# raulmur/ORB_SLAM2

Measured on NVIDIA H100. Metric: stereo frames/sec (ORB extract L+R + ComputeStereoMatches, KITTI-shaped 1242x375 @2000 kpts), higher is better.
Workload: dtype u8

## Files before the change

### orb_slam2_b200/csrc/borb_host.cu

```cuda
#include <cmath>
#include <cstdarg>
#include <cstdio>
#include <algorithm>
#include <cstdlib>
#include <cstring>

#include "borb_internal.h"

namespace borb {

static thread_local std::string tl_error;
void set_error(const char* fmt, ...) {
    char buf[512];
    va_list ap;
    va_start(ap, fmt);
    vsnprintf(buf, sizeof(buf), fmt, ap);
    va_end(ap);
    tl_error = buf;
}

bool allow_max_smem(const void* func) {
    static std::mutex mu;
    static std::vector<std::pair<const void*, int>> done;
    int dev = 0;
// ... 66 lines not shown
        int r = 2 * dst - 2 - (dst + k);
        if (r < 0) r = 0;
        for (int j = 0; j < 4; j++) out.push_back(out[first + (size_t)r * 4 + j]);
    }
    if (((out.size() - first) / 4) & 1) for (int j = 0; j < 4; j++) out.push_back(0);
}

bool resize_window_table(const std::vector<int16_t>& tabs, size_t xtab_first, int n_entries, std::vector<int16_t>& out) {
    bool ok = true;
    for (int gq = 0; gq < n_entries; gq += 4) {
        int lo = 1 << 30, hi = 0;
        for (int i = 0; i < 4; i++) {
            const int ofs = tabs[xtab_first + (size_t)(gq + i) * 4];
            lo = std::min(lo, ofs); hi = std::max(hi, ofs);
        }
        const int base = lo & ~3;
        if (hi + 1 - base > 11) ok = false;
        for (int i = 0; i < 4; i++) {
            const int16_t* e = &tabs[xtab_first + (size_t)(gq + i) * 4];
            const int pos = e[0] - base;
            int s1 = 0, s2 = 0x10;
            if (pos <= 6) s1 = pos | ((pos + 1) << 4);
            else if (pos == 7) { s1 = 7; s2 = 0x40; }
            else { const int q = (pos - 8) + 4; s2 = q | ((q + 1) << 4); }
            out.push_back(e[1]);
            out.push_back(e[2]);
            out.push_back((int16_t)base);
            out.push_back((int16_t)((s1 | (s2 << 8)) & 0x7FFF));
        }
    }
    return ok;
}

const int8_t kPattern[1024] = {
#include "orb_pattern.inc"
};

borb_status build_geometry(borb_extractor* e, int w, int h, std::vector<int16_t>& tabs) {
    Geometry& g = e->geom;
    std::memset(&g, 0, sizeof(g));
    const int L = e->cfg.n_levels;
    g.nlevels = L; g.w = w; g.h = h;
    g.fast_mode = e->fast_mode;
    g.ini_th = e->cfg.ini_th_fast < 0 ? 0 : (e->cfg.ini_th_fast > 255 ? 255 : e->cfg.ini_th_fast);
    g.min_th = e->cfg.min_th_fast < 0 ? 0 : (e->cfg.min_th_fast > 255 ? 255 : e->cfg.min_th_fast);
    for (int i = 0; i < 16; i++) g.umax[i] = e->umax[i];
    unsigned pyr_off = 0, cand_off = 0;
    int blk = 0, sel_off = 0, btile = 0;
    tabs.clear();
    for (int l = 0; l < L; l++) {
        LevelGeom& v = g.lv[l];
        v.w = cv_round_f((float)w * e->inv_scale[l]);
        v.h = cv_round_f((float)h * e->inv_scale[l]);
        const float width = (float)(v.w - 2 * MIN_BORDER), height = (float)(v.h - 2 * MIN_BORDER);
        v.nCols = (int)(width / 30.f);
        v.nRows = (int)(height / 30.f);
        if (v.nCols < 1 || v.nRows < 1) {
            set_error("level %d is %dx%d: too small for the 30-px FAST cell grid (reference divides by zero)", l, v.w, v.h);
            return BORB_ERR_UNSUPPORTED;
        }
        v.wCell = (int)std::ceil(width / v.nCols);
        v.hCell = (int)std::ceil(height / v.nRows);
        v.pitch = align_up(v.w + 8, 128);
        v.pyr_off = pyr_off;
        pyr_off += (unsigned)v.pitch * v.h;
        v.cellsPerBlk = FAST_TILE_W / v.wCell > 0 ? FAST_TILE_W / v.wCell : 1;
        v.rowsPerBlk = fast_rows_per_blk(v.nRows, v.hCell);
        v.blkCols = (v.nCols + v.cellsPerBlk - 1) / v.cellsPerBlk;
        v.blkBase = blk;
        blk += v.blkCols * ((v.nRows + v.rowsPerBlk - 1) / v.rowsPerBlk);
        v.cand_off = cand_off;
        v.cand_cap = v.nCols * v.nRows * ((v.wCell + 1) / 2) * ((v.hCell + 1) / 2);
        cand_off += (unsigned)align_up(v.cand_cap, 32);
        v.quota = e->per_level[l];
        v.nIni = (int)std::round(width / height);
        if (v.nIni < 1) { set_error("level %d aspect ratio gives zero quadtree roots (reference divides by zero)", l); return BORB_ERR_UNSUPPORTED; }
        v.hX = width / v.nIni;
        v.node_cap = (v.quota > 4 * v.nIni ? v.quota : 4 * v.nIni) + 3;
        v.node_cap = align_up(v.node_cap + 1, 4);
        v.sel_off = sel_off;
        sel_off += v.node_cap;
        v.scale = e->scale[l];
        v.inv_scale = e->inv_scale[l];
        v.patch_size = (float)(int)(PATCH * e->scale[l]);
        g.blur_base[l] = btile;
        btile += ((v.w + BLUR_TILE_W - 1) / BLUR_TILE_W) * ((v.h + BLUR_TILE_H - 1) / BLUR_TILE_H);
        if (l > 0) {
            const int wpad = (v.w + 8 + 3) & ~3;
            v.xtab_off = (unsigned)(tabs.size() / 4);
            resize_table(g.lv[l - 1].w, v.w, true, wpad - v.w, tabs);
            v.ytab_off = (unsigned)(tabs.size() / 4);
            resize_table(g.lv[l - 1].h, v.h, false, 0, tabs);
            v.xwin_off = (unsigned)(tabs.size() / 4);
            std::vector<int16_t> win;
            v.x_windowed = resize_window_table(tabs, (size_t)v.xtab_off * 4, wpad, win) ? 1 : 0;
            tabs.insert(tabs.end(), win.begin(), win.end());
        }
        if (quadtree_smem_bytes(v.node_cap) > 200 * 1024) {
            set_error("per-level quota %d exceeds the quadtree kernel's shared-memory envelope", v.quota);
            return BORB_ERR_UNSUPPORTED;
        }
    }
    g.blur_base[L] = btile;
    g.blur_tiles = btile;
    g.fast_blocks = blk;
    g.pyr_image_stride = (unsigned)align_up((int)pyr_off, g.lv[0].pitch);
    g.cand_image_stride = cand_off;
    g.sel_image_stride = sel_off;
    if (sel_off >= 65536) { set_error("keypoint capacity %d exceeds 65535", sel_off); return BORB_ERR_UNSUPPORTED; }
    return BORB_OK;
}

void free_workspace(Workspace& ws) {
    cudaFree(ws.pyr); cudaFree(ws.blur); cudaFree(ws.cand); cudaFree(ws.cand_cnt); cudaFree(ws.pnode); cudaFree(ws.sel);
    cudaFree(ws.sel_cnt); cudaFree(ws.kps); cudaFree(ws.desc); cudaFree(ws.nkp); cudaFree(ws.u_right); cudaFree(ws.depth);
    cudaFree(ws.sad); cudaFree(ws.tabs); cudaFree(ws.brief_slots); cudaFree(ws.pair_idx); cudaFree(ws.st_bins); cudaFree(ws.st_recs); cudaFree(ws.stage);
    free(ws.fast_tmaps); cudaFree(ws.fast_tiles);
    ws = Workspace();
}

borb_status ensure(borb_extractor* e, int w, int h, int n_images) {
    if (w < 1 || h < 1 || w > BORB_MAX_DIM || h > BORB_MAX_DIM) { set_error("image size %dx%d outside [1,%d]", w, h, BORB_MAX_DIM); return BORB_ERR_UNSUPPORTED; }
    BORB_CUDA(cudaSetDevice(e->device));
    const bool same_shape = e->have_geom && e->geom.w == w && e->geom.h == h;
    if (same_shape && e->ws.max_images >= n_images) return BORB_OK;
    BORB_CUDA(cudaStreamSynchronize(e->stream));
    std::vector<int16_t> tabs;
    e->have_geom = false;
    e->last_n_images = 0;
    e->last_stereo_pairs = 0;
    borb_status st = build_geometry(e, w, h, tabs);
    if (st != BORB_OK) return st;
    size_t n = (size_t)(n_images > 2 ? n_images : 2);
    if (same_shape && (size_t)e->ws.max_images > n) n = (size_t)e->ws.max_images;
    free_workspace(e->ws);
    if (e->h_counts) { cudaFreeHost(e->h_counts); e->h_counts = nullptr; }
    e->pair_cache.clear();
    const Geometry& g = e->geom;
    Workspace& ws = e->ws;
    BORB_CUDA(cudaMalloc(&ws.pyr, n * g.pyr_image_stride + 256));
    BORB_CUDA(cudaMalloc(&ws.blur, n * g.pyr_image_stride + 256));
    BORB_CUDA(cudaMalloc(&ws.cand, n * g.cand_image_stride * sizeof(uint32_t)));
    BORB_CUDA(cudaMalloc(&ws.pnode, n * g.cand_image_stride * sizeof(int)));
    BORB_CUDA(cudaMalloc(&ws.cand_cnt, n * g.nlevels * sizeof(int)));
    BORB_CUDA(cudaMalloc(&ws.sel, n * g.sel_image_stride * sizeof(uint32_t)));
    BORB_CUDA(cudaMalloc(&ws.sel_cnt, n * g.nlevels * sizeof(int)));
    BORB_CUDA(cudaMalloc(&ws.kps, n * g.sel_image_stride * sizeof(borb_keypoint)));
    BORB_CUDA(cudaMalloc(&ws.desc, n * g.sel_image_stride * 32));
    BORB_CUDA(cudaMalloc(&ws.nkp, n * sizeof(int)));
    BORB_CUDA(cudaMalloc(&ws.u_right, n * g.sel_image_stride * sizeof(float)));
    BORB_CUDA(cudaMalloc(&ws.depth, n * g.sel_image_stride * sizeof(float)));
    BORB_CUDA(cudaMalloc(&ws.sad, n * g.sel_image_stride * sizeof(int)));
    BORB_CUDA(cudaMalloc(&ws.pair_idx, n * 2 * sizeof(int)));
    BORB_CUDA(cudaMalloc(&ws.st_bins, n * stereo_bins_bytes_per_pair()));
    BORB_CUDA(cudaMalloc(&ws.st_recs, n * (size_t)stereo_rec_stride(g) * stereo_rec_bytes()));
    BORB_CUDA(cudaMalloc(&ws.tabs, (tabs.size() + 4) * sizeof(int16_t)));
    BORB_CUDA(cudaMemcpy(ws.tabs, tabs.data(), tabs.size() * sizeof(int16_t), cudaMemcpyHostToDevice));
    const std::vector<uint32_t>& slots = brief_slot_table();
    BORB_CUDA(cudaMalloc(&ws.brief_slots, slots.size() * sizeof(uint32_t)));
    BORB_CUDA(cudaMemcpy(ws.brief_slots, slots.data(), slots.size() * sizeof(uint32_t), cudaMemcpyHostToDevice));
    BORB_CUDA(cudaMemset(ws.nkp, 0, n * sizeof(int)));
    BORB_CUDA(cudaMallocHost(&e->h_counts, n * 2 * sizeof(int)));
    ws.max_images = (int)n;
    ws.fast_tmaps = malloc(fast_tmaps_bytes());
    if ((st = build_fast_tmaps(g, ws, ws.fast_tmaps)) != BORB_OK) return st;
    if ((st = build_fast_tiles(g, ws)) != BORB_OK) return st;
    e->have_geom = true;
    return BORB_OK;
}

void drain_timing(borb_extractor* e);
void begin_step(borb_extractor* e) {
    if (!e->timing) return;
    if (e->ev.empty()) {
        e->ev.resize((size_t)borb_extractor::EV_RING * 9);
        for (auto& x : e->ev) cudaEventCreate(&x);
    }
    if (e->ev_pending >= borb_extractor::EV_RING) {
        cudaStreamSynchronize(e->stream);
        drain_timing(e);
    }
    e->ev_slot = (e->ev_slot + 1) % borb_extractor::EV_RING;
    e->ev_mask[e->ev_slot] = 0;
    e->ev_pending++;
}
void mark(borb_extractor* e, int i) {
    if (!e->timing || e->ev.empty()) return;
    cudaEventRecord(e->ev[(size_t)e->ev_slot * 9 + i], e->stream);
    e->ev_mask[e->ev_slot] |= 1u << i;
}
void drain_timing(borb_extractor* e) {
    const int R = borb_extractor::EV_RING;
    for (int k = e->ev_pending - 1; k >= 0; k--) {
        const int slot = ((e->ev_slot - k) % R + R) % R;
        const unsigned m = e->ev_mask[slot];
        for (int i = 0; i < 8; i++) {
            float ms = 0.f;
            if (m & (1u << i)) {
                int j = i + 1;
                while (j < 9 && !(m & (1u << j))) j++;
                if (j < 9 && cudaEventElapsedTime(&ms, e->ev[(size_t)slot * 9 + i], e->ev[(size_t)slot * 9 + j]) != cudaSuccess) { ms = 0.f; cudaGetLastError(); }
            }
            e->stage_ms[i] = ms;
            e->stage_sum_ms[i] += ms;
        }
        e->stage_steps++;
    }
    e->ev_pending = 0;
}

borb_status enqueue_extract(borb_extractor* e, int n) {
    const Geometry& g = e->geom;
    Workspace& ws = e->ws;
    cudaStream_t s = e->stream;
    BORB_CUDA(cudaMemsetAsync(ws.cand_cnt, 0, (size_t)n * g.nlevels * sizeof(int), s));
    mark(e, 1);
    e->launches += launch_pyramid(g, ws, n, s);
    mark(e, 2);
    e->launches += launch_fast(g, ws, n, s);
    mark(e, 3);
    e->launches += launch_quadtree(g, ws, n, s);
    mark(e, 4);
    e->launches += launch_blur(g, ws, n, s);
    mark(e, 5);
    e->launches += launch_describe(g, ws, n, s);
    mark(e, 6);
    BORB_CUDA(cudaGetLastError());
    e->last_n_images = n;
    e->last_stereo_pairs = 0;
    return BORB_OK;
}

borb_status rectified_size(borb_extractor* e, int w, int h, int* gw, int* gh) {
    if (!e->d_map[0][0]) return BORB_OK;
    if (w != e->map_src_w || h != e->map_src_h) {
        set_error("rectification maps were built for %dx%d raw frames, got %dx%d", e->map_src_w, e->map_src_h, w, h);
        return BORB_ERR_INVALID_ARG;
    }
    *gw = e->map_dst_w; *gh = e->map_dst_h;
    return BORB_OK;
}

borb_status upload_slots(borb_extractor* e, const uint8_t* const* slots, int n, int w, int h, int stride, bool stereo_pairs = false) {
    const Geometry& g = e->geom;
    const int ch = e->in_channels;
    if (stride < w * ch) { set_error("stride %d smaller than a row of %d %d-channel pixels", stride, w, ch); return BORB_ERR_INVALID_ARG; }
    const size_t img_bytes = (size_t)stride * h;
    bool contiguous = n > 1 || ch > 1 || e->d_map[0][0] != nullptr;
    for (int k = 0; k < n; k++) {
        if (!slots[k]) { set_error("image %d is NULL", k); return BORB_ERR_INVALID_ARG; }
        if (slots[k] != slots[0] + (size_t)k * img_bytes) contiguous = false;
    }
    auto need_stage = [&](size_t need) -> borb_status {
        if (e->ws.stage_bytes < need) {
            BORB_CUDA(cudaStreamSynchronize(e->stream));
            cudaFree(e->ws.stage);
            e->ws.stage = nullptr; e->ws.stage_bytes = 0;
            BORB_CUDA(cudaMalloc(&e->ws.stage, need));
            e->ws.stage_bytes = need;
        }
        return BORB_OK;
    };
    if (e->d_map[0][0]) {
        if (ch != 1) { set_error("rectification maps apply to CV_8UC1 frames"); return BORB_ERR_UNSUPPORTED; }
        const size_t src_img = contiguous ? img_bytes : (size_t)w * h;
        const int src_stride = contiguous ? stride : w;
        borb_status st = need_stage(src_img * n);
        if (st != BORB_OK) return st;
        if (contiguous) BORB_CUDA(cudaMemcpyAsync(e->ws.stage, slots[0], src_img * n, cudaMemcpyHostToDevice, e->stream));
        else
            for (int k = 0; k < n; k++)
                BORB_CUDA(cudaMemcpy2DAsync(e->ws.stage + (size_t)k * src_img, w, slots[k], stride, w, h, cudaMemcpyHostToDevice, e->stream));
        e->launches += launch_repack_remap(g, e->ws, e->ws.stage, src_stride, src_img, w, h, e->d_map[0][0], e->d_map[0][1],
                                           stereo_pairs ? e->d_map[1][0] : nullptr, stereo_pairs ? e->d_map[1][1] : nullptr, n, e->stream);
        return BORB_OK;
    }
    if (contiguous) {
        const size_t need = img_bytes * n;
        borb_status st = need_stage(need);
        if (st != BORB_OK) return st;
        BORB_CUDA(cudaMemcpyAsync(e->ws.stage, slots[0], need, cudaMemcpyHostToDevice, e->stream));
        if (ch == 1) e->launches += launch_repack(g, e->ws, e->ws.stage, stride, img_bytes, n, e->stream);
        else e->launches += launch_repack_color(g, e->ws, e->ws.stage, stride, img_bytes, ch, e->in_rgb, n, e->stream);
        return BORB_OK;
    }
    if (ch > 1) {
        const size_t row = (size_t)w * ch;
        borb_status st = need_stage(row * h * n);
        if (st != BORB_OK) return st;
        for (int k = 0; k < n; k++)
            BORB_CUDA(cudaMemcpy2DAsync(e->ws.stage + (size_t)k * row * h, row, slots[k], stride, row, h, cudaMemcpyHostToDevice, e->stream));
        e->launches += launch_repack_color(g, e->ws, e->ws.stage, (int)row, row * h, ch, e->in_rgb, n, e->stream);
        return BORB_OK;
    }
    for (int k = 0; k < n; k++) {
        uint8_t* dst = e->ws.pyr + (size_t)k * g.pyr_image_stride + g.lv[0].pyr_off;
        BORB_CUDA(cudaMemcpy2DAsync(dst, g.lv[0].pitch, slots[k], stride, w, h, cudaMemcpyHostToDevice, e->stream));
    }
    return BORB_OK;
}

borb_status upload_device(borb_extractor* e, const uint8_t* d_gray, int n, int w, int h, size_t pitch, size_t image_stride) {
    const Geometry& g = e->geom;
    cudaMemcpy3DParms p = {};
    p.srcPtr = make_cudaPitchedPtr((void*)d_gray, pitch, w, image_stride / pitch);
    p.dstPtr = make_cudaPitchedPtr(e->ws.pyr + g.lv[0].pyr_off, g.lv[0].pitch, w, g.pyr_image_stride / g.lv[0].pitch);
    if (image_stride % pitch == 0 && g.pyr_image_stride % g.lv[0].pitch == 0) {
// ... 548 lines not shown
```

### orb_slam2_b200/csrc/borb_internal.h

```cpp
#pragma once
#include <cuda_runtime.h>
#include <stdint.h>

#include <mutex>
#include <string>
#include <vector>

#include "../../include/borb.h"

namespace borb {

constexpr int EDGE = 19;
constexpr int PATCH = 31;
constexpr int HALF_PATCH = 15;
constexpr int MIN_BORDER = 16;
constexpr int TH_HIGH = 100;
constexpr int TH_LOW = 50;
constexpr int BLUR_TILE_W = 120;
constexpr int BLUR_TILE_H = 64;
constexpr int FAST_TILE_W = 124;
constexpr int FAST_H_BAND = 64;

__host__ __device__ inline int fast_rows_per_blk(int nRows, int hCell) {
    const int r = FAST_H_BAND / hCell;
    return r < 1 ? 1 : (r > nRows ? nRows : r);
}
__host__ __device__ inline int fast_box_rows(int rowsPerBlk, int hCell) { return rowsPerBlk * hCell + 6; }

__host__ __device__ inline uint32_t pack_xys(int x, int y, int s) { return (uint32_t)x | ((uint32_t)y << 12) | ((uint32_t)s << 24); }
__host__ __device__ inline int xys_x(uint32_t v) { return (int)(v & 0xFFFu); }
__host__ __device__ inline int xys_y(uint32_t v) { return (int)((v >> 12) & 0xFFFu); }
__host__ __device__ inline int xys_s(uint32_t v) { return (int)(v >> 24); }

struct LevelGeom {
    int w, h;
    int pitch;
    unsigned pyr_off;
    int nCols, nRows, wCell, hCell;
    int cellsPerBlk;
    int rowsPerBlk;
    int blkCols;
    int blkBase;
    unsigned cand_off;
    int cand_cap;
    int quota;
    int nIni;
    float hX;
    int node_cap;
    int sel_off;
    float scale;
    float inv_scale;
    float patch_size;
    unsigned xtab_off, ytab_off;
    unsigned xwin_off;
    int x_windowed;
};

struct Geometry {
    int nlevels;
    int w, h;
    int ini_th, min_th;
    int fast_mode;
    int fast_blocks;
    unsigned pyr_image_stride;
    unsigned cand_image_stride;
    int sel_image_stride;
    int blur_tiles;
    int blur_base[BORB_MAX_LEVELS + 1];
    int umax[16];
    LevelGeom lv[BORB_MAX_LEVELS];
};

struct Workspace {
    int max_images = 0;
    uint8_t* pyr = nullptr;
    uint8_t* blur = nullptr;
    uint32_t* cand = nullptr;
    int* cand_cnt = nullptr;
    int* pnode = nullptr;
    uint32_t* sel = nullptr;
    int* sel_cnt = nullptr;
    borb_keypoint* kps = nullptr;
    uint8_t* desc = nullptr;
    int* nkp = nullptr;
    float* u_right = nullptr;
    float* depth = nullptr;
    int* sad = nullptr;
    int16_t* tabs = nullptr;
    uint32_t* brief_slots = nullptr;
    int* pair_idx = nullptr;
    int* st_bins = nullptr;
    void* st_recs = nullptr;
    uint8_t* stage = nullptr;
    size_t stage_bytes = 0;
    void* fast_tmaps = nullptr;
    void* fast_tiles = nullptr;
    int fast_n_tiles = 0;
};

constexpr int BRIEF_BINS = 32;
const std::vector<uint32_t>& brief_slot_table();

void set_error(const char* fmt, ...);
bool allow_max_smem(const void* func);
#define BORB_CUDA(call)                                                                             \
    do {                                                                                            \
        cudaError_t _e = (call);                                                                    \
        if (_e != cudaSuccess) {                                                                    \
            borb::set_error("%s failed: %s (%s:%d)", #call, cudaGetErrorString(_e), __FILE__, __LINE__); \
            return (_e == cudaErrorNoDevice || _e == cudaErrorInsufficientDriver) ? BORB_ERR_NO_DEVICE : BORB_ERR_CUDA; \
        }                                                                                           \
    } while (0)

int launch_repack_remap(const Geometry& g, const Workspace& ws, const uint8_t* stage, int src_stride, size_t src_image_bytes, int src_w,
                        int src_h, const float* mx0, const float* my0, const float* mx1, const float* my1, int n_images, cudaStream_t s);
int launch_repack_color(const Geometry& g, const Workspace& ws, const uint8_t* stage, int src_stride, size_t src_image_bytes, int channels,
                        int rgb, int n_images, cudaStream_t s);
int launch_repack(const Geometry& g, const Workspace& ws, const uint8_t* stage, int src_stride, size_t src_image_bytes,
                  int n_images, cudaStream_t s);
int launch_pyramid(const Geometry& g, const Workspace& ws, int n_images, cudaStream_t s);
int launch_fast(const Geometry& g, const Workspace& ws, int n_images, cudaStream_t s);
int launch_quadtree(const Geometry& g, const Workspace& ws, int n_images, cudaStream_t s);
int launch_blur(const Geometry& g, const Workspace& ws, int n_images, cudaStream_t s);
int launch_describe(const Geometry& g, const Workspace& ws, int n_images, cudaStream_t s);

struct StereoView {
    const uint8_t* pyr;
    const borb_keypoint* kps;
    const uint8_t* desc;
    const int* nkp;
    unsigned pyr_image_stride;
    int kp_image_stride;
};
int launch_stereo(const Geometry& g, const StereoView& L, const StereoView& R, const int* d_pair_idx, int n_pairs,
                  float bf, float b, float* d_u_right, float* d_depth, int* d_sad, int out_stride, int* d_bins, void* d_recs,
                  cudaStream_t s);
int stereo_rec_stride(const Geometry& g);
size_t stereo_bins_bytes_per_pair();
size_t stereo_rec_bytes();
size_t quadtree_smem_bytes(int node_cap);
borb_status build_fast_tmaps(const Geometry& g, const Workspace& ws, void* out_tmaps);
borb_status build_fast_tiles(const Geometry& g, Workspace& ws);
size_t fast_tmaps_bytes();

}

struct borb_extractor {
    borb_extractor_cfg cfg;
    int device = 0;
    cudaStream_t stream = nullptr;
    std::vector<float> scale, inv_scale, sigma2, inv_sigma2;
    std::vector<int> per_level;
    int umax[16];
    bool have_geom = false;
    borb::Geometry geom;
    borb::Workspace ws;
    int last_n_images = 0;
    int last_stereo_pairs = 0;
    int in_channels = 1;
    int in_rgb = 1;
    float* d_map[2][2] = {{nullptr, nullptr}, {nullptr, nullptr}};
    int map_src_w = 0, map_src_h = 0, map_dst_w = 0, map_dst_h = 0;
    int fast_mode = 0;
    uint64_t launches = 0;
    static constexpr int EV_RING = 128;
    bool timing = false;
    std::vector<cudaEvent_t> ev;
    unsigned ev_mask[EV_RING] = {};
    int ev_slot = 0;
    int ev_pending = 0;
    float stage_ms[8] = {};
    double stage_sum_ms[8] = {};
    uint64_t stage_steps = 0;
    int* h_counts = nullptr;
    std::vector<int> pair_cache;
};
```

### orb_slam2_b200/csrc/k_stereo.cu

```cuda
#include "borb_internal.h"

namespace borb {

namespace {

__device__ __forceinline__ int hamming256(const uint4 a0, const uint4 a1, const uint4* __restrict__ b) {
    const uint4 b0 = b[0], b1 = b[1];
    return __popc(a0.x ^ b0.x) + __popc(a0.y ^ b0.y) + __popc(a0.z ^ b0.z) + __popc(a0.w ^ b0.w) +
           __popc(a1.x ^ b1.x) + __popc(a1.y ^ b1.y) + __popc(a1.z ^ b1.z) + __popc(a1.w ^ b1.w);
}

}

constexpr int SBIN_SHIFT = 3;
constexpr int SBIN_MAX = 512;
struct __align__(16) RightRec { int iR; int band; int octave; float x; };

__global__ void __launch_bounds__(256) stereo_bin_kernel(const __grid_constant__ Geometry g, StereoView Rv,
                                                         const int* __restrict__ pair_idx, int* __restrict__ bin_start,
                                                         RightRec* __restrict__ recs, int rec_stride) {
    __shared__ int cnt[SBIN_MAX + 1];
    __shared__ int wsum[40];
    const int pair = blockIdx.x, tid = threadIdx.x;
    const int imR = pair_idx[2 * pair + 1];
    const int nR = Rv.nkp[imR];
    const int nb = min((g.h >> SBIN_SHIFT) + 1, SBIN_MAX);
    const borb_keypoint* kR = Rv.kps + (size_t)imR * Rv.kp_image_stride;
    for (int i = tid; i <= nb; i += 256) cnt[i] = 0;
    __syncthreads();
    for (int i = tid; i < nR; i += 256) {
        const borb_keypoint kr = kR[i];
        const float r = __fmul_rn(2.0f, g.lv[kr.octave].scale);
        const int maxr = (int)ceilf(__fadd_rn(kr.y, r)), minr = (int)floorf(__fsub_rn(kr.y, r));
        const int b0 = max(minr, 0) >> SBIN_SHIFT, b1 = min(min(maxr, g.h - 1) >> SBIN_SHIFT, nb - 1);
        for (int b = b0; b <= b1; b++) atomicAdd(&cnt[b], 1);
    }
    __syncthreads();
    {
        const int lane = tid & 31, w = tid >> 5;
        const int i0 = 2 * tid, i1 = 2 * tid + 1;
        const int c0 = i0 < nb ? cnt[i0] : 0, c1 = i1 < nb ? cnt[i1] : 0;
        int incl = c0 + c1;
#pragma unroll
        for (int off = 1; off < 32; off <<= 1) {
            const int t = __shfl_up_sync(0xFFFFFFFFu, incl, off);
            if (lane >= off) incl += t;
        }
        if (lane == 31) wsum[w] = incl;
        __syncthreads();
        if (w == 0) {
            int v = lane < 8 ? wsum[lane] : 0, inc2 = v;
#pragma unroll
            for (int off = 1; off < 8; off <<= 1) {
                const int t = __shfl_up_sync(0xFFFFFFFFu, inc2, off);
                if (lane >= off) inc2 += t;
            }
            if (lane < 8) wsum[8 + lane] = inc2 - v;
            if (lane == 7) wsum[16] = inc2;
        }
        __syncthreads();
        const int base = wsum[8 + w] + incl - (c0 + c1);
        if (i0 < nb) cnt[i0] = base;
        if (i1 < nb) cnt[i1] = base + c0;
        if (tid == 0) cnt[nb] = wsum[16];
        __syncthreads();
    }
    int* bs = bin_start + (size_t)pair * (SBIN_MAX + 1);
    for (int i = tid; i <= nb; i += 256) bs[i] = cnt[i];
    __syncthreads();
    RightRec* out = recs + (size_t)pair * rec_stride;
    for (int i = tid; i < nR; i += 256) {
        const borb_keypoint kr = kR[i];
        const float r = __fmul_rn(2.0f, g.lv[kr.octave].scale);
        const int maxr = (int)ceilf(__fadd_rn(kr.y, r)), minr = (int)floorf(__fsub_rn(kr.y, r));
        const int b0 = max(minr, 0) >> SBIN_SHIFT, b1 = min(min(maxr, g.h - 1) >> SBIN_SHIFT, nb - 1);
        RightRec rec;
        rec.iR = i; rec.band = (minr & 0xFFFF) | (maxr << 16); rec.octave = kr.octave; rec.x = kr.x;
        for (int b = b0; b <= b1; b++) {
            const int pos = atomicAdd(&cnt[b], 1);
            if (pos < rec_stride) out[pos] = rec;
        }
    }
}

__global__ void __launch_bounds__(256, 6) stereo_match_kernel(const __grid_constant__ Geometry g, StereoView Lv, StereoView Rv,
                                                           const int* __restrict__ pair_idx, float bf, float b,
                                                           float* __restrict__ u_right, float* __restrict__ depth,
                                                           int* __restrict__ sad, int out_stride,
                                                           const int* __restrict__ bin_start, const RightRec* __restrict__ recs,
                                                           int rec_stride) {
    const int pair = blockIdx.y;
    const int imL = pair_idx[2 * pair], imR = pair_idx[2 * pair + 1];
    const int lane = threadIdx.x & 31;
    const int iL = blockIdx.x * (blockDim.x >> 5) + (threadIdx.x >> 5);
    const int nL = Lv.nkp[imL], nR = Rv.nkp[imR];
    if (iL >= nL) return;
    const size_t o = (size_t)pair * out_stride + iL;
    const borb_keypoint* kL = Lv.kps + (size_t)imL * Lv.kp_image_stride;
    const borb_keypoint* kR = Rv.kps + (size_t)imR * Rv.kp_image_stride;
    const uint8_t* dL = Lv.desc + (size_t)imL * Lv.kp_image_stride * 32;
    const uint8_t* dR = Rv.desc + (size_t)imR * Rv.kp_image_stride * 32;

    float uR_out = -1.0f, depth_out = -1.0f;
    int sad_out = -1;

    const borb_keypoint kp = kL[iL];
    const int levelL = kp.octave;
    const float vL = kp.y, uL = kp.x;
    const float maxD = __fdiv_rn(bf, b);
    const float minU = __fsub_rn(uL, maxD), maxU = uL;
    const int row = (int)vL;
    const uint4 a0 = reinterpret_cast<const uint4*>(dL + (size_t)iL * 32)[0];
    const uint4 a1 = reinterpret_cast<const uint4*>(dL + (size_t)iL * 32)[1];
    unsigned best = ((unsigned)TH_HIGH << 16);
    if (!(maxU < 0) && row >= 0 && row < g.h) {
        const int nb = min((g.h >> SBIN_SHIFT) + 1, SBIN_MAX);
        const int bin = min(row >> SBIN_SHIFT, nb - 1);
        const int* bs = bin_start + (size_t)pair * (SBIN_MAX + 1);
        const int e0 = bs[bin], e1 = min(bs[bin + 1], rec_stride);
        const RightRec* rr = recs + (size_t)pair * rec_stride;
        for (int e = e0 + lane; e < e1; e += 32) {
            const RightRec rc = rr[e];
            const int minr = (int)(short)(rc.band & 0xFFFF), maxr = rc.band >> 16;
            if (row < minr || row > maxr) continue;
            if (rc.octave < levelL - 1 || rc.octave > levelL + 1) continue;
            if (rc.x >= minU && rc.x <= maxU) {
                const int dist = hamming256(a0, a1, reinterpret_cast<const uint4*>(dR + (size_t)rc.iR * 32));
                const unsigned key = ((unsigned)dist << 16) | (unsigned)rc.iR;
                best = min(best, key);
            }
        }
    }
#pragma unroll
    for (int off = 16; off > 0; off >>= 1) best = min(best, __shfl_xor_sync(0xFFFFFFFFu, best, off));
    const int bestDist = (int)(best >> 16);
    const int thOrbDist = (TH_HIGH + TH_LOW) / 2;
    if (bestDist < thOrbDist) {
        const int bestIdxR = (int)(best & 0xFFFFu);
        const float uR0 = kR[bestIdxR].x;
        const LevelGeom& LG = g.lv[levelL];
        const float sf = LG.inv_scale;
        const int scaleduL = (int)roundf(__fmul_rn(kp.x, sf));
        const int scaledvL = (int)roundf(__fmul_rn(kp.y, sf));
        const int scaleduR0 = (int)roundf(__fmul_rn(uR0, sf));
        const int w = 5, Lh = 5;
        const int iniu = scaleduR0 + Lh - w, endu = scaleduR0 + Lh + w + 1;
        const bool ok = !(iniu < 0 || endu >= LG.w) && scaleduR0 - Lh - w >= 0 && scaledvL - w >= 0 &&
                        scaledvL + w < LG.h && scaleduL - w >= 0 && scaleduL + w < LG.w;
        if (ok) {
            const uint8_t* IL = Lv.pyr + (size_t)imL * Lv.pyr_image_stride + LG.pyr_off;
            const uint8_t* IR = Rv.pyr + (size_t)imR * Rv.pyr_image_stride + LG.pyr_off;
            const int cL = IL[(size_t)scaledvL * LG.pitch + scaleduL];
            int il[4];
            int offs[4];
#pragma unroll
            for (int k = 0; k < 4; k++) {
                const int e = lane + 32 * k;
                if (e < 121) {
                    const int yy = e / 11, xx = e - yy * 11;
                    offs[k] = (scaledvL - w + yy) * LG.pitch + (xx - w);
                    il[k] = (int)IL[offs[k] + scaleduL] - cL;
                } else { offs[k] = -1; il[k] = 0; }
            }
            int bestD = 0x7FFFFFFF, bestinc = 0;
            int dists[11];
#pragma unroll
            for (int inc = -5; inc <= 5; inc++) {
                const int uc = scaleduR0 + inc;
                const int cR = IR[(size_t)scaledvL * LG.pitch + uc];
                int s = 0;
#pragma unroll
                for (int k = 0; k < 4; k++)
                    if (offs[k] >= 0) s += abs(il[k] - ((int)IR[offs[k] + uc] - cR));
#pragma unroll
                for (int off = 16; off > 0; off >>= 1) s += __shfl_xor_sync(0xFFFFFFFFu, s, off);
                dists[inc + 5] = s;
                if (s < bestD) { bestD = s; bestinc = inc; }
            }
            if (!(bestinc == -Lh || bestinc == Lh)) {
                float d1 = 0.f, d2 = 0.f, d3 = 0.f;
#pragma unroll
                for (int i = 1; i < 10; i++)
                    if (i == bestinc + 5) { d1 = (float)dists[i - 1]; d2 = (float)dists[i]; d3 = (float)dists[i + 1]; }
                const float num = __fsub_rn(d1, d3);
                const float den = __fmul_rn(2.0f, __fsub_rn(__fadd_rn(d1, d3), __fmul_rn(2.0f, d2)));
                const float deltaR = __fdiv_rn(num, den);
                if (!(deltaR < -1.f || deltaR > 1.f)) {
                    float bestuR = __fmul_rn(LG.scale, __fadd_rn(__fadd_rn((float)scaleduR0, (float)bestinc), deltaR));
                    float disparity = __fsub_rn(uL, bestuR);
                    if (disparity >= 0.f && disparity < maxD) {
                        if (disparity <= 0.f) {
                            disparity = 0.01f;
                            bestuR = (float)((double)uL - 0.01);
                        }
                        depth_out = __fdiv_rn(bf, disparity);
                        uR_out = bestuR;
                        sad_out = bestD;
                    }
                }
            }
        }
    }
    if (lane == 0) {
        u_right[o] = uR_out;
        depth[o] = depth_out;
        sad[o] = sad_out;
    }
}

__global__ void __launch_bounds__(256) stereo_median_kernel(StereoView Lv, const int* __restrict__ pair_idx,
                                                            float* __restrict__ u_right, float* __restrict__ depth,
                                                            const int* __restrict__ sad, int out_stride) {
    __shared__ int hist[256];
    __shared__ int sel[3];
    const int pair = blockIdx.x;
    const int nL = Lv.nkp[pair_idx[2 * pair]];
    const size_t o = (size_t)pair * out_stride;
    const int tid = threadIdx.x;
    hist[tid] = 0;
    __syncthreads();
    int cnt = 0;
    for (int i = tid; i < nL; i += 256) {
        const int d = sad[o + i];
        if (d >= 0) { atomicAdd(&hist[min(d >> 8, 255)], 1); cnt++; }
    }
    __shared__ int tot;
    if (tid == 0) tot = 0;
    __syncthreads();
    if (cnt) atomicAdd(&tot, cnt);
    __syncthreads();
    const int n = tot;
    if (n == 0) return;
    const int kth = n / 2;
    if (tid == 0) {
        int acc = 0, bin = 0;
        for (; bin < 256; bin++) { if (acc + hist[bin] > kth) break; acc += hist[bin]; }
        sel[0] = bin; sel[1] = kth - acc;
    }
    __syncthreads();
    const int hiBin = sel[0], rem = sel[1];
    __syncthreads();
    hist[tid] = 0;
    __syncthreads();
    for (int i = tid; i < nL; i += 256) {
        const int d = sad[o + i];
        if (d >= 0 && min(d >> 8, 255) == hiBin) atomicAdd(&hist[d & 255], 1);
    }
    __syncthreads();
    if (tid == 0) {
        int acc = 0, bin = 0;
        for (; bin < 256; bin++) { if (acc + hist[bin] > rem) break; acc += hist[bin]; }
        sel[2] = (hiBin << 8) | bin;
    }
    __syncthreads();
    const float median = (float)sel[2];
    const float thDist = __fmul_rn(1.5f * 1.4f, median);
    for (int i = tid; i < nL; i += 256) {
        const int d = sad[o + i];
        if (d >= 0 && !((float)d < thDist)) { u_right[o + i] = -1.0f; depth[o + i] = -1.0f; }
    }
}

int stereo_rec_stride(const Geometry& g) {
    const int band = 2 * (int)ceilf(2.0f * g.lv[g.nlevels - 1].scale) + 3;
    return g.sel_image_stride * ((band >> SBIN_SHIFT) + 2);
}
size_t stereo_bins_bytes_per_pair() { return (size_t)(SBIN_MAX + 1) * sizeof(int); }
size_t stereo_rec_bytes() { return sizeof(RightRec); }

int launch_stereo(const Geometry& g, const StereoView& L, const StereoView& R, const int* d_pair_idx, int n_pairs,
                  float bf, float b, float* d_u_right, float* d_depth, int* d_sad, int out_stride, int* d_bins, void* d_recs,
                  cudaStream_t s) {
    const int rec_stride = stereo_rec_stride(g);
    stereo_bin_kernel<<<n_pairs, 256, 0, s>>>(g, R, d_pair_idx, d_bins, reinterpret_cast<RightRec*>(d_recs), rec_stride);
    dim3 grid((g.sel_image_stride + 7) / 8, n_pairs);
    stereo_match_kernel<<<grid, 256, 0, s>>>(g, L, R, d_pair_idx, bf, b, d_u_right, d_depth, d_sad, out_stride, d_bins,
                                             reinterpret_cast<const RightRec*>(d_recs), rec_stride);
    stereo_median_kernel<<<n_pairs, 256, 0, s>>>(L, d_pair_idx, d_u_right, d_depth, d_sad, out_stride);
    return 3;
}

}
```

Before: 43940.

## Bin left keypoints by row and stage right candidates in shared memory per bin

The bin kernel now also bins the left keypoints by row band, producing a sorted index list. The match kernel launches one block per row bin instead of one warp per left keypoint. Each block stages that bin's right-keypoint records and descriptors in shared memory once, and all left keypoints in the bin reuse them, replacing repeated global descriptor gathers. This costs a larger shared-memory footprint, a lower occupancy hint, and possible load imbalance across bins; a global-memory fallback handles bins with more than 512 candidates.

```diff
diff --git a/orb_slam2_b200/csrc/borb_host.cu b/orb_slam2_b200/csrc/borb_host.cu
--- a/orb_slam2_b200/csrc/borb_host.cu
+++ b/orb_slam2_b200/csrc/borb_host.cu
@@ -242,7 +242,7 @@
     BORB_CUDA(cudaMalloc(&ws.depth, n * g.sel_image_stride * sizeof(float)));
     BORB_CUDA(cudaMalloc(&ws.sad, n * g.sel_image_stride * sizeof(int)));
     BORB_CUDA(cudaMalloc(&ws.pair_idx, n * 2 * sizeof(int)));
-    BORB_CUDA(cudaMalloc(&ws.st_bins, n * stereo_bins_bytes_per_pair()));
+    BORB_CUDA(cudaMalloc(&ws.st_bins, n * stereo_bins_bytes_per_pair(g)));
     BORB_CUDA(cudaMalloc(&ws.st_recs, n * (size_t)stereo_rec_stride(g) * stereo_rec_bytes()));
     BORB_CUDA(cudaMalloc(&ws.tabs, (tabs.size() + 4) * sizeof(int16_t)));
     BORB_CUDA(cudaMemcpy(ws.tabs, tabs.data(), tabs.size() * sizeof(int16_t), cudaMemcpyHostToDevice));
diff --git a/orb_slam2_b200/csrc/borb_internal.h b/orb_slam2_b200/csrc/borb_internal.h
--- a/orb_slam2_b200/csrc/borb_internal.h
+++ b/orb_slam2_b200/csrc/borb_internal.h
@@ -136,7 +136,7 @@
                   float bf, float b, float* d_u_right, float* d_depth, int* d_sad, int out_stride, int* d_bins, void* d_recs,
                   cudaStream_t s);
 int stereo_rec_stride(const Geometry& g);
-size_t stereo_bins_bytes_per_pair();
+size_t stereo_bins_bytes_per_pair(const Geometry& g);
 size_t stereo_rec_bytes();
 size_t quadtree_smem_bytes(int node_cap);
 borb_status build_fast_tmaps(const Geometry& g, const Workspace& ws, void* out_tmaps);
diff --git a/orb_slam2_b200/csrc/k_stereo.cu b/orb_slam2_b200/csrc/k_stereo.cu
--- a/orb_slam2_b200/csrc/k_stereo.cu
+++ b/orb_slam2_b200/csrc/k_stereo.cu
@@ -4,8 +4,7 @@
 
 namespace {
 
-__device__ __forceinline__ int hamming256(const uint4 a0, const uint4 a1, const uint4* __restrict__ b) {
-    const uint4 b0 = b[0], b1 = b[1];
+__device__ __forceinline__ int hamming256(const uint4 a0, const uint4 a1, const uint4 b0, const uint4 b1) {
     return __popc(a0.x ^ b0.x) + __popc(a0.y ^ b0.y) + __popc(a0.z ^ b0.z) + __popc(a0.w ^ b0.w) +
            __popc(a1.x ^ b1.x) + __popc(a1.y ^ b1.y) + __popc(a1.z ^ b1.z) + __popc(a1.w ^ b1.w);
 }
@@ -14,63 +13,97 @@
 
 constexpr int SBIN_SHIFT = 3;
 constexpr int SBIN_MAX = 512;
+constexpr int SBIN_STRIDE = SBIN_MAX + 1;
+constexpr int SREC_CAP = 512;
 struct __align__(16) RightRec { int iR; int band; int octave; float x; };
 
-__global__ void __launch_bounds__(256) stereo_bin_kernel(const __grid_constant__ Geometry g, StereoView Rv,
-                                                         const int* __restrict__ pair_idx, int* __restrict__ bin_start,
-                                                         RightRec* __restrict__ recs, int rec_stride) {
+__host__ __device__ __forceinline__ int stereo_nbins(int h) { return min((h >> SBIN_SHIFT) + 1, SBIN_MAX); }
+
+__host__ __device__ __forceinline__ int stereo_bins_ints(int kp_stride) { return 2 * SBIN_STRIDE + kp_stride; }
+
+__device__ __forceinline__ void scan_bins(int* cnt, int nb, int* wsum) {
+    const int tid = threadIdx.x, lane = tid & 31, w = tid >> 5;
+    const int i0 = 2 * tid, i1 = 2 * tid + 1;
+    const int c0 = i0 < nb ? cnt[i0] : 0, c1 = i1 < nb ? cnt[i1] : 0;
+    int incl = c0 + c1;
+#pragma unroll
+    for (int off = 1; off < 32; off <<= 1) {
+        const int t = __shfl_up_sync(0xFFFFFFFFu, incl, off);
+        if (lane >= off) incl += t;
+    }
+    if (lane == 31) wsum[w] = incl;
+    __syncthreads();
+    if (w == 0) {
+        int v = lane < 8 ? wsum[lane] : 0, inc2 = v;
+#pragma unroll
+        for (int off = 1; off < 8; off <<= 1) {
+            const int t = __shfl_up_sync(0xFFFFFFFFu, inc2, off);
+            if (lane >= off) inc2 += t;
+        }
+        if (lane < 8) wsum[8 + lane] = inc2 - v;
+        if (lane == 7) wsum[16] = inc2;
+    }
+    __syncthreads();
+    const int base = wsum[8 + w] + incl - (c0 + c1);
+    if (i0 < nb) cnt[i0] = base;
+    if (i1 < nb) cnt[i1] = base + c0;
+    if (tid == 0) cnt[nb] = wsum[16];
+    __syncthreads();
+}
+
+__global__ void __launch_bounds__(256) stereo_bin_kernel(const __grid_constant__ Geometry g, StereoView Lv, StereoView Rv,
+                                                         const int* __restrict__ pair_idx, int* __restrict__ bins, int bins_stride,
+                                                         RightRec* __restrict__ recs, int rec_stride, float* __restrict__ u_right,
+                                                         float* __restrict__ depth, int* __restrict__ sad, int out_stride) {
     __shared__ int cnt[SBIN_MAX + 1];
     __shared__ int wsum[40];
     const int pair = blockIdx.x, tid = threadIdx.x;
-    const int imR = pair_idx[2 * pair + 1];
-    const int nR = Rv.nkp[imR];
-    const int nb = min((g.h >> SBIN_SHIFT) + 1, SBIN_MAX);
-    const borb_keypoint* kR = Rv.kps + (size_t)imR * Rv.kp_image_stride;
+    const bool left = blockIdx.y == 1;
+    const int nb = stereo_nbins(g.h);
+    const int im = pair_idx[2 * pair + (left ? 0 : 1)];
+    const int n = (left ? Lv.nkp : Rv.nkp)[im];
+    const borb_keypoint* kp = (left ? Lv.kps : Rv.kps) + (size_t)im * (left ? Lv.kp_image_stride : Rv.kp_image_stride);
+    int* bs = bins + (size_t)pair * bins_stride + (left ? SBIN_STRIDE : 0);
     for (int i = tid; i <= nb; i += 256) cnt[i] = 0;
     __syncthreads();
-    for (int i = tid; i < nR; i += 256) {
-        const borb_keypoint kr = kR[i];
-        const float r = __fmul_rn(2.0f, g.lv[kr.octave].scale);
-        const int maxr = (int)ceilf(__fadd_rn(kr.y, r)), minr = (int)floorf(__fsub_rn(kr.y, r));
-        const int b0 = max(minr, 0) >> SBIN_SHIFT, b1 = min(min(maxr, g.h - 1) >> SBIN_SHIFT, nb - 1);
-        for (int b = b0; b <= b1; b++) atomicAdd(&cnt[b], 1);
-    }
-    __syncthreads();
-    {
-        const int lane = tid & 31, w = tid >> 5;
-        const int i0 = 2 * tid, i1 = 2 * tid + 1;
-        const int c0 = i0 < nb ? cnt[i0] : 0, c1 = i1 < nb ? cnt[i1] : 0;
-        int incl = c0 + c1;
-#pragma unroll
-        for (int off = 1; off < 32; off <<= 1) {
-            const int t = __shfl_up_sync(0xFFFFFFFFu, incl, off);
-            if (lane >= off) incl += t;
-        }
-        if (lane == 31) wsum[w] = incl;
-        __syncthreads();
-        if (w == 0) {
-            int v = lane < 8 ? wsum[lane] : 0, inc2 = v;
-#pragma unroll
-            for (int off = 1; off < 8; off <<= 1) {
-                const int t = __shfl_up_sync(0xFFFFFFFFu, inc2, off);
-                if (lane >= off) inc2 += t;
+    if (left) {
+        for (int i = tid; i < n; i += 256) {
+            const borb_keypoint k = kp[i];
+            const int row = (int)k.y;
+            if (!(k.x < 0) && row >= 0 && row < g.h) atomicAdd(&cnt[min(row >> SBIN_SHIFT, nb - 1)], 1);
+        }
+    } else {
+        for (int i = tid; i < n; i += 256) {
+            const borb_keypoint kr = kp[i];
+            const float r = __fmul_rn(2.0f, g.lv[kr.octave].scale);
+            const int maxr = (int)ceilf(__fadd_rn(kr.y, r)), minr = (int)floorf(__fsub_rn(kr.y, r));
+            const int b0 = max(minr, 0) >> SBIN_SHIFT, b1 = min(min(maxr, g.h - 1) >> SBIN_SHIFT, nb - 1);
+            for (int b = b0; b <= b1; b++) atomicAdd(&cnt[b], 1);
+        }
+    }
+    __syncthreads();
+    scan_bins(cnt, nb, wsum);
+    for (int i = tid; i <= nb; i += 256) bs[i] = cnt[i];
+    __syncthreads();
+    if (left) {
+        int* lidx = bs + SBIN_STRIDE;
+        const size_t o = (size_t)pair * out_stride;
+        for (int i = tid; i < n; i += 256) {
+            const borb_keypoint k = kp[i];
+            const int row = (int)k.y;
+            if (!(k.x < 0) && row >= 0 && row < g.h) {
+                lidx[atomicAdd(&cnt[min(row >> SBIN_SHIFT, nb - 1)], 1)] = i;
+            } else {
+                u_right[o + i] = -1.0f;
+                depth[o + i] = -1.0f;
+                sad[o + i] = -1;
             }
-            if (lane < 8) wsum[8 + lane] = inc2 - v;
-            if (lane == 7) wsum[16] = inc2;
-        }
-        __syncthreads();
-        const int base = wsum[8 + w] + incl - (c0 + c1);
-        if (i0 < nb) cnt[i0] = base;
-        if (i1 < nb) cnt[i1] = base + c0;
-        if (tid == 0) cnt[nb] = wsum[16];
-        __syncthreads();
-    }
-    int* bs = bin_start + (size_t)pair * (SBIN_MAX + 1);
-    for (int i = tid; i <= nb; i += 256) bs[i] = cnt[i];
-    __syncthreads();
+        }
+        return;
+    }
     RightRec* out = recs + (size_t)pair * rec_stride;
-    for (int i = tid; i < nR; i += 256) {
-        const borb_keypoint kr = kR[i];
+    for (int i = tid; i < n; i += 256) {
+        const borb_keypoint kr = kp[i];
         const float r = __fmul_rn(2.0f, g.lv[kr.octave].scale);
         const int maxr = (int)ceilf(__fadd_rn(kr.y, r)), minr = (int)floorf(__fsub_rn(kr.y, r));
         const int b0 = max(minr, 0) >> SBIN_SHIFT, b1 = min(min(maxr, g.h - 1) >> SBIN_SHIFT, nb - 1);
@@ -83,128 +116,160 @@
     }
 }
 
-__global__ void __launch_bounds__(256, 6) stereo_match_kernel(const __grid_constant__ Geometry g, StereoView Lv, StereoView Rv,
+template <bool STAGED>
+__device__ __forceinline__ unsigned bin_search(const RightRec* __restrict__ rr, const uint4* __restrict__ sd0,
+                                               const uint4* __restrict__ sd1, const uint4* __restrict__ dR, int nrec, int lane,
+                                               int row, int levelL, float minU, float maxU, uint4 a0, uint4 a1, float& uR0) {
+    unsigned best = ((unsigned)TH_HIGH << 16);
+    float bx = 0.f;
+    for (int e = lane; e < nrec; e += 32) {
+        const RightRec rc = rr[e];
+        const int minr = (int)(short)(rc.band & 0xFFFF), maxr = rc.band >> 16;
+        if (row < minr || row > maxr) continue;
+        if (rc.octave < levelL - 1 || rc.octave > levelL + 1) continue;
+        if (rc.x >= minU && rc.x <= maxU) {
+            const int dist = STAGED ? hamming256(a0, a1, sd0[e], sd1[e])
+                                    : hamming256(a0, a1, dR[2 * (size_t)rc.iR], dR[2 * (size_t)rc.iR + 1]);
+            const unsigned key = ((unsigned)dist << 16) | (unsigned)rc.iR;
+            if (key < best) { best = key; bx = rc.x; }
+        }
+    }
+    unsigned wbest = best;
+#pragma unroll
+    for (int off = 16; off > 0; off >>= 1) wbest = min(wbest, __shfl_xor_sync(0xFFFFFFFFu, wbest, off));
+    const unsigned owner = __ballot_sync(0xFFFFFFFFu, best == wbest);
+    uR0 = __shfl_sync(0xFFFFFFFFu, bx, __ffs(owner) - 1);
+    return wbest;
+}
+
+__global__ void __launch_bounds__(256, 5) stereo_match_kernel(const __grid_constant__ Geometry g, StereoView Lv, StereoView Rv,
                                                            const int* __restrict__ pair_idx, float bf, float b,
                                                            float* __restrict__ u_right, float* __restrict__ depth,
                                                            int* __restrict__ sad, int out_stride,
-                                                           const int* __restrict__ bin_start, const RightRec* __restrict__ recs,
-                                                           int rec_stride) {
-    const int pair = blockIdx.y;
+                                                           const int* __restrict__ bins, int bins_stride,
+                                                           const RightRec* __restrict__ recs, int rec_stride) {
+    __shared__ RightRec srec[SREC_CAP];
+    __shared__ uint4 sd0[SREC_CAP], sd1[SREC_CAP];
+    __shared__ uint4 sA0[256], sA1[256];
+    __shared__ int sIL[256], sOctL[256];
+    __shared__ float sXL[256], sYL[256];
+    const int pair = blockIdx.y, bin = blockIdx.x;
+    const int* bsR = bins + (size_t)pair * bins_stride;
+    const int* bsL = bsR + SBIN_STRIDE;
+    const int* lidx = bsL + SBIN_STRIDE;
+    const int l0 = bsL[bin], l1 = bsL[bin + 1];
+    if (l0 >= l1) return;
+    const int tid = threadIdx.x, lane = tid & 31, warp = tid >> 5;
     const int imL = pair_idx[2 * pair], imR = pair_idx[2 * pair + 1];
-    const int lane = threadIdx.x & 31;
-    const int iL = blockIdx.x * (blockDim.x >> 5) + (threadIdx.x >> 5);
-    const int nL = Lv.nkp[imL], nR = Rv.nkp[imR];
-    if (iL >= nL) return;
-    const size_t o = (size_t)pair * out_stride + iL;
     const borb_keypoint* kL = Lv.kps + (size_t)imL * Lv.kp_image_stride;
-    const borb_keypoint* kR = Rv.kps + (size_t)imR * Rv.kp_image_stride;
-    const uint8_t* dL = Lv.desc + (size_t)imL * Lv.kp_image_stride * 32;
-    const uint8_t* dR = Rv.desc + (size_t)imR * Rv.kp_image_stride * 32;
-
-    float uR_out = -1.0f, depth_out = -1.0f;
-    int sad_out = -1;
-
-    const borb_keypoint kp = kL[iL];
-    const int levelL = kp.octave;
-    const float vL = kp.y, uL = kp.x;
+    const uint4* dL = reinterpret_cast<const uint4*>(Lv.desc + (size_t)imL * Lv.kp_image_stride * 32);
+    const uint4* dR = reinterpret_cast<const uint4*>(Rv.desc + (size_t)imR * Rv.kp_image_stride * 32);
+    const int r0 = bsR[bin], r1 = min(bsR[bin + 1], rec_stride);
+    const int nrec = max(r1 - r0, 0);
+    const bool staged = nrec <= SREC_CAP;
+    const RightRec* rr = recs + (size_t)pair * rec_stride + r0;
+
     const float maxD = __fdiv_rn(bf, b);
-    const float minU = __fsub_rn(uL, maxD), maxU = uL;
-    const int row = (int)vL;
-    const uint4 a0 = reinterpret_cast<const uint4*>(dL + (size_t)iL * 32)[0];
-    const uint4 a1 = reinterpret_cast<const uint4*>(dL + (size_t)iL * 32)[1];
-    unsigned best = ((unsigned)TH_HIGH << 16);
-    if (!(maxU < 0) && row >= 0 && row < g.h) {
-        const int nb = min((g.h >> SBIN_SHIFT) + 1, SBIN_MAX);
-        const int bin = min(row >> SBIN_SHIFT, nb - 1);
-        const int* bs = bin_start + (size_t)pair * (SBIN_MAX + 1);
-        const int e0 = bs[bin], e1 = min(bs[bin + 1], rec_stride);
-        const RightRec* rr = recs + (size_t)pair * rec_stride;
-        for (int e = e0 + lane; e < e1; e += 32) {
-            const RightRec rc = rr[e];
-            const int minr = (int)(short)(rc.band & 0xFFFF), maxr = rc.band >> 16;
-            if (row < minr || row > maxr) continue;
-            if (rc.octave < levelL - 1 || rc.octave > levelL + 1) continue;
-            if (rc.x >= minU && rc.x <= maxU) {
-                const int dist = hamming256(a0, a1, reinterpret_cast<const uint4*>(dR + (size_t)rc.iR * 32));
-                const unsigned key = ((unsigned)dist << 16) | (unsigned)rc.iR;
-                best = min(best, key);
+    const int thOrbDist = (TH_HIGH + TH_LOW) / 2;
+    for (int base = l0; base < l1; base += 256) {
+        if (base != l0) __syncthreads();
+        if (base + tid < l1) {
+            const int i = lidx[base + tid];
+            const borb_keypoint& k = kL[i];
+            sIL[tid] = i; sXL[tid] = k.x; sYL[tid] = k.y; sOctL[tid] = k.octave;
+            sA0[tid] = dL[2 * (size_t)i]; sA1[tid] = dL[2 * (size_t)i + 1];
+        }
+        if (base == l0 && staged) {
+            for (int e = tid; e < nrec; e += 256) {
+                const RightRec rc = rr[e];
+                srec[e] = rc;
+                sd0[e] = dR[2 * (size_t)rc.iR];
+                sd1[e] = dR[2 * (size_t)rc.iR + 1];
             }
         }
-    }
-#pragma unroll
-    for (int off = 16; off > 0; off >>= 1) best = min(best, __shfl_xor_sync(0xFFFFFFFFu, best, off));
-    const int bestDist = (int)(best >> 16);
-    const int thOrbDist = (TH_HIGH + TH_LOW) / 2;
-    if (bestDist < thOrbDist) {
-        const int bestIdxR = (int)(best & 0xFFFFu);
-        const float uR0 = kR[bestIdxR].x;
-        const LevelGeom& LG = g.lv[levelL];
-        const float sf = LG.inv_scale;
-        const int scaleduL = (int)roundf(__fmul_rn(kp.x, sf));
-        const int scaledvL = (int)roundf(__fmul_rn(kp.y, sf));
-        const int scaleduR0 = (int)roundf(__fmul_rn(uR0, sf));
-        const int w = 5, Lh = 5;
-        const int iniu = scaleduR0 + Lh - w, endu = scaleduR0 + Lh + w + 1;
-        const bool ok = !(iniu < 0 || endu >= LG.w) && scaleduR0 - Lh - w >= 0 && scaledvL - w >= 0 &&
-                        scaledvL + w < LG.h && scaleduL - w >= 0 && scaleduL + w < LG.w;
-        if (ok) {
-            const uint8_t* IL = Lv.pyr + (size_t)imL * Lv.pyr_image_stride + LG.pyr_off;
-            const uint8_t* IR = Rv.pyr + (size_t)imR * Rv.pyr_image_stride + LG.pyr_off;
-            const int cL = IL[(size_t)scaledvL * LG.pitch + scaleduL];
-            int il[4];
-            int offs[4];
-#pragma unroll
-            for (int k = 0; k < 4; k++) {
-                const int e = lane + 32 * k;
-                if (e < 121) {
-                    const int yy = e / 11, xx = e - yy * 11;
-                    offs[k] = (scaledvL - w + yy) * LG.pitch + (xx - w);
-                    il[k] = (int)IL[offs[k] + scaleduL] - cL;
-                } else { offs[k] = -1; il[k] = 0; }
-            }
-            int bestD = 0x7FFFFFFF, bestinc = 0;
-            int dists[11];
-#pragma unroll
-            for (int inc = -5; inc <= 5; inc++) {
-                const int uc = scaleduR0 + inc;
-                const int cR = IR[(size_t)scaledvL * LG.pitch + uc];
-                int s = 0;
-#pragma unroll
-                for (int k = 0; k < 4; k++)
-                    if (offs[k] >= 0) s += abs(il[k] - ((int)IR[offs[k] + uc] - cR));
-#pragma unroll
-                for (int off = 16; off > 0; off >>= 1) s += __shfl_xor_sync(0xFFFFFFFFu, s, off);
-                dists[inc + 5] = s;
-                if (s < bestD) { bestD = s; bestinc = inc; }
-            }
-            if (!(bestinc == -Lh || bestinc == Lh)) {
-                float d1 = 0.f, d2 = 0.f, d3 = 0.f;
-#pragma unroll
-                for (int i = 1; i < 10; i++)
-                    if (i == bestinc + 5) { d1 = (float)dists[i - 1]; d2 = (float)dists[i]; d3 = (float)dists[i + 1]; }
-                const float num = __fsub_rn(d1, d3);
-                const float den = __fmul_rn(2.0f, __fsub_rn(__fadd_rn(d1, d3), __fmul_rn(2.0f, d2)));
-                const float deltaR = __fdiv_rn(num, den);
-                if (!(deltaR < -1.f || deltaR > 1.f)) {
-                    float bestuR = __fmul_rn(LG.scale, __fadd_rn(__fadd_rn((float)scaleduR0, (float)bestinc), deltaR));
-                    float disparity = __fsub_rn(uL, bestuR);
-                    if (disparity >= 0.f && disparity < maxD) {
-                        if (disparity <= 0.f) {
-                            disparity = 0.01f;
-                            bestuR = (float)((double)uL - 0.01);
+        __syncthreads();
+        const int cnt = min(256, l1 - base);
+        for (int j = warp; j < cnt; j += 8) {
+            const int i = sIL[j], levelL = sOctL[j];
+            const float uL = sXL[j], vL = sYL[j];
+            const uint4 q0 = sA0[j], q1 = sA1[j];
+            const float minU = __fsub_rn(uL, maxD), maxU = uL;
+            const int row = (int)vL;
+            float uR0;
+            const unsigned best = staged ? bin_search<true>(srec, sd0, sd1, dR, nrec, lane, row, levelL, minU, maxU, q0, q1, uR0)
+                                         : bin_search<false>(rr, nullptr, nullptr, dR, nrec, lane, row, levelL, minU, maxU, q0, q1, uR0);
+            float uR_out = -1.0f, depth_out = -1.0f;
+            int sad_out = -1;
+            const int bestDist = (int)(best >> 16);
+            if (bestDist < thOrbDist) {
+                const LevelGeom& LG = g.lv[levelL];
+                const float sf = LG.inv_scale;
+                const int scaleduL = (int)roundf(__fmul_rn(uL, sf));
+                const int scaledvL = (int)roundf(__fmul_rn(vL, sf));
+                const int scaleduR0 = (int)roundf(__fmul_rn(uR0, sf));
+                const int w = 5, Lh = 5;
+                const int iniu = scaleduR0 + Lh - w, endu = scaleduR0 + Lh + w + 1;
+                const bool ok = !(iniu < 0 || endu >= LG.w) && scaleduR0 - Lh - w >= 0 && scaledvL - w >= 0 &&
+                                scaledvL + w < LG.h && scaleduL - w >= 0 && scaleduL + w < LG.w;
+                if (ok) {
+                    const uint8_t* IL = Lv.pyr + (size_t)imL * Lv.pyr_image_stride + LG.pyr_off;
+                    const uint8_t* IR = Rv.pyr + (size_t)imR * Rv.pyr_image_stride + LG.pyr_off;
+                    const int cL = IL[(size_t)scaledvL * LG.pitch + scaleduL];
+                    int il[4];
+                    int offs[4];
+#pragma unroll
+                    for (int k = 0; k < 4; k++) {
+                        const int e = lane + 32 * k;
+                        if (e < 121) {
+                            const int yy = e / 11, xx = e - yy * 11;
+                            offs[k] = (scaledvL - w + yy) * LG.pitch + (xx - w);
+                            il[k] = (int)IL[offs[k] + scaleduL] - cL;
+                        } else { offs[k] = -1; il[k] = 0; }
+                    }
+                    int bestD = 0x7FFFFFFF, bestinc = 0, prev = 0, dPrev = 0, dNext = 0;
+                    bool wantNext = false;
+#pragma unroll
+                    for (int inc = -5; inc <= 5; inc++) {
+                        const int uc = scaleduR0 + inc;
+                        const int cR = IR[(size_t)scaledvL * LG.pitch + uc];
+                        int s = 0;
+#pragma unroll
+                        for (int k = 0; k < 4; k++)
+                            if (offs[k] >= 0) s += abs(il[k] - ((int)IR[offs[k] + uc] - cR));
+#pragma unroll
+                        for (int off = 16; off > 0; off >>= 1) s += __shfl_xor_sync(0xFFFFFFFFu, s, off);
+                        if (wantNext) { dNext = s; wantNext = false; }
+                        if (s < bestD) { bestD = s; bestinc = inc; dPrev = prev; wantNext = true; }
+                        prev = s;
+                    }
+                    if (!(bestinc == -Lh || bestinc == Lh)) {
+                        const float d1 = (float)dPrev, d2 = (float)bestD, d3 = (float)dNext;
+                        const float num = __fsub_rn(d1, d3);
+                        const float den = __fmul_rn(2.0f, __fsub_rn(__fadd_rn(d1, d3), __fmul_rn(2.0f, d2)));
+                        const float deltaR = __fdiv_rn(num, den);
+                        if (!(deltaR < -1.f || deltaR > 1.f)) {
+                            float bestuR = __fmul_rn(LG.scale, __fadd_rn(__fadd_rn((float)scaleduR0, (float)bestinc), deltaR));
+                            float disparity = __fsub_rn(uL, bestuR);
+                            if (disparity >= 0.f && disparity < maxD) {
+                                if (disparity <= 0.f) {
+                                    disparity = 0.01f;
+                                    bestuR = (float)((double)uL - 0.01);
+                                }
+                                depth_out = __fdiv_rn(bf, disparity);
+                                uR_out = bestuR;
+                                sad_out = bestD;
+                            }
                         }
-                        depth_out = __fdiv_rn(bf, disparity);
-                        uR_out = bestuR;
-                        sad_out = bestD;
                     }
                 }
             }
-        }
-    }
-    if (lane == 0) {
-        u_right[o] = uR_out;
-        depth[o] = depth_out;
-        sad[o] = sad_out;
+            if (lane == 0) {
+                const size_t o = (size_t)pair * out_stride + i;
+                u_right[o] = uR_out;
+                depth[o] = depth_out;
+                sad[o] = sad_out;
+            }
+        }
     }
 }
 
@@ -265,17 +330,19 @@
     const int band = 2 * (int)ceilf(2.0f * g.lv[g.nlevels - 1].scale) + 3;
     return g.sel_image_stride * ((band >> SBIN_SHIFT) + 2);
 }
-size_t stereo_bins_bytes_per_pair() { return (size_t)(SBIN_MAX + 1) * sizeof(int); }
+size_t stereo_bins_bytes_per_pair(const Geometry& g) { return (size_t)stereo_bins_ints(g.sel_image_stride) * sizeof(int); }
 size_t stereo_rec_bytes() { return sizeof(RightRec); }
 
 int launch_stereo(const Geometry& g, const StereoView& L, const StereoView& R, const int* d_pair_idx, int n_pairs,
                   float bf, float b, float* d_u_right, float* d_depth, int* d_sad, int out_stride, int* d_bins, void* d_recs,
                   cudaStream_t s) {
     const int rec_stride = stereo_rec_stride(g);
-    stereo_bin_kernel<<<n_pairs, 256, 0, s>>>(g, R, d_pair_idx, d_bins, reinterpret_cast<RightRec*>(d_recs), rec_stride);
-    dim3 grid((g.sel_image_stride + 7) / 8, n_pairs);
-    stereo_match_kernel<<<grid, 256, 0, s>>>(g, L, R, d_pair_idx, bf, b, d_u_right, d_depth, d_sad, out_stride, d_bins,
-                                             reinterpret_cast<const RightRec*>(d_recs), rec_stride);
+    const int bins_stride = stereo_bins_ints(g.sel_image_stride);
+    RightRec* recs = reinterpret_cast<RightRec*>(d_recs);
+    stereo_bin_kernel<<<dim3(n_pairs, 2), 256, 0, s>>>(g, L, R, d_pair_idx, d_bins, bins_stride, recs, rec_stride, d_u_right, d_depth,
+                                                       d_sad, out_stride);
+    stereo_match_kernel<<<dim3(stereo_nbins(g.h), n_pairs), 256, 0, s>>>(g, L, R, d_pair_idx, bf, b, d_u_right, d_depth, d_sad,
+                                                                         out_stride, d_bins, bins_stride, recs, rec_stride);
     stereo_median_kernel<<<n_pairs, 256, 0, s>>>(L, d_pair_idx, d_u_right, d_depth, d_sad, out_stride);
     return 3;
 }
```

Result: faster. 44750 (median of 6 runs) (+1.8%).
